# showlab/EgoVLP

Hardware: AMD Instinct MI355X
Metric: clip-pairs/sec (whole node), 4f/224^2 ViT-B + 32-tok text, B=32/GPU, train step (fwd+gather+EgoNCE+bwd+AdamW) (higher is better)
Workload: dtype fp16 (every Linear and both attentions of the video blocks, forward and backward) + bf16 (patch embedding, text tower, heads) MFMA operands, fp32 accumulate

## Files before the change

### egovlp_amd/csrc/block.hip

```cpp
#include <hip/hip_runtime.h>

#include <algorithm>

#include "layer_call.h"

namespace {

struct FwdLayout {
  int64_t n3_hi, n3_lo, mean3, rstd3, qkvt_hi, qkvt_lo, at_hi, at_lo, lse_t, work_t;
  int64_t tr, n1_hi, n1_lo, mean1, rstd1, qkvs_hi, qkvs_lo, as_hi, as_lo, lse_s, work_s;
  int64_t sr, n2_hi, n2_lo, mean2, rstd2, h_hi, h_lo, z;
  int64_t n3_bf, n1_bf, n2_bf, h_bf;
  int64_t n1c, mean1c, rstd1c, qc, oc, n2c, hc;
  int64_t total;
};

struct Geo {
  int64_t M, S, D, Hd;
  int P, Pb;
};

inline bool is_train(const egv_block_geom& g) { return (g.train & 1) != 0; }
inline bool is_tail(const egv_block_geom& g) { return (g.train & 2) != 0; }

Geo geo_of(const egv_block_geom& g) {
  Geo o;
  o.S = 1 + (int64_t)g.T * g.n;
  o.M = (int64_t)g.B * o.S;
  o.D = g.D;
  o.Hd = g.Hd;
  o.P = g.fwd_passes;
  o.Pb = g.bwd_passes;
  return o;
}

bool geom_ok(const egv_block_geom& g) {
  if (g.B <= 0 || g.T <= 0 || g.n <= 0 || g.H <= 0 || g.D != g.H * 64 || g.Hd <= 0 || g.D % 32 || g.Hd % 32) return false;
  if (g.fwd_passes < 1 || g.fwd_passes > 3 || (g.bwd_passes != 1 && g.bwd_passes != 3 && g.bwd_passes != 4)) return false;
  if (g.bwd_passes == 3 && g.fwd_passes != 3) return false;
  if (g.bwd_passes == 4 && g.fwd_passes != 2) return false;
  if (g.train < 0 || g.train > 3) return false;
  if (g.fwd_passes == 2 && (g.bwd_passes == 3 || (is_train(g) && !g.z_bf16))) return false;
  if (g.f16_single < 0 || g.f16_single > 15 || (g.f16_single && g.fwd_passes != 2)) return false;
  return true;
}

FwdLayout fwd_layout(const egv_block_geom& g) {
  const Geo o = geo_of(g);
  const bool lo = o.P != 1;
  const bool h16 = o.Pb == 4;
  const bool bf = o.P == 2 && is_train(g) && !h16;
  const bool tail = is_tail(g);
  FwdLayout L;
  Bump b;
  auto plane = [&](int64_t cols) { return b.take(o.M * cols * 2); };
  auto plane_lo = [&](int64_t cols) { return lo ? b.take(o.M * cols * 2) : (int64_t)-1; };
  auto plane_bf = [&](int64_t cols) { return bf ? b.take(o.M * cols * 2) : (int64_t)-1; };
  const bool q1 = (g.f16_single & 4) != 0;
  L.n3_hi = plane(o.D); L.n3_lo = q1 ? (int64_t)-1 : plane_lo(o.D);
  L.mean3 = b.take(o.M * 4); L.rstd3 = b.take(o.M * 4);
  L.qkvt_hi = plane(3 * o.D); L.qkvt_lo = plane_lo(3 * o.D);
  const bool a1p = h16 && (g.f16_single & 8);
  L.at_hi = plane(o.D); L.at_lo = a1p ? (int64_t)-1 : plane_lo(o.D);
  L.lse_t = b.take((int64_t)g.B * g.H * o.S * 4);
  L.work_t = b.take(egv_divided_attn_fwd_work_floats(g.B, g.T, g.n, g.H, 1) * 4);
  L.tr = b.take(o.M * o.D * 4);
  L.n1_hi = plane(o.D); L.n1_lo = q1 ? (int64_t)-1 : plane_lo(o.D);
  L.mean1 = b.take(o.M * 4); L.rstd1 = b.take(o.M * 4);
  L.n1c = L.mean1c = L.rstd1c = L.qc = L.oc = L.n2c = L.hc = -1;
  if (tail) {
    const int64_t B = g.B;
    L.qkvs_hi = plane(2 * o.D); L.qkvs_lo = plane_lo(2 * o.D);
    L.as_hi = L.as_lo = L.work_s = L.n2_hi = L.n2_lo = L.h_hi = L.h_lo = L.n2_bf = L.h_bf = -1;
    L.lse_s = b.take(B * g.H * 4);
// ... 236 lines not shown
  const FwdLayout F = fwd_layout(g);
  const BwdLayout L = bwd_layout(g, io.wgrad_ksplit);
  int64_t goff[18], gtot;
  grad_layout(g, goff, gtot);
  const int32_t M = (int32_t)o.M, D = (int32_t)o.D, Hd = (int32_t)o.Hd;
  for (int i = 0; i < (tail ? 3 : 6); ++i)
    if (!p.wt_hi[i] || (Pb == 3 && !p.wt_lo[i])) return EGV_ERR_ARG;
  if (Pb == 3 && (!io.dx_lo || (io.g_hi && !io.g_lo))) return EGV_ERR_ARG;
  const bool h16 = Pb == 4;
  constexpr float A1_INV = 1.0f / (1.0f - 0.015625f);
  const char* FA = (const char*)io.fwd_arena;
  char* A = (char*)io.bwd_arena;
  hipStream_t main_s = (hipStream_t)stream;
  const bool x2 = o.P == 2 && !h16;
  const egv_bf16 *n3_hi, *n3_lo, *at_hi, *at_lo, *n1_hi, *n1_lo, *as_hi, *as_lo, *n2_hi, *n2_lo, *h_hi, *h_lo, *qt_hi, *qt_lo, *qs_hi, *qs_lo;
  saved_planes(FA, Pb, x2 ? F.n3_bf : F.n3_hi, F.n3_lo, n3_hi, n3_lo);
  saved_planes(FA, Pb, F.at_hi, F.at_lo, at_hi, at_lo);
  saved_planes(FA, Pb, x2 ? F.n1_bf : F.n1_hi, F.n1_lo, n1_hi, n1_lo);
  saved_planes(FA, Pb, F.as_hi, F.as_lo, as_hi, as_lo);
  saved_planes(FA, Pb, x2 ? F.n2_bf : F.n2_hi, F.n2_lo, n2_hi, n2_lo);
  saved_planes(FA, Pb, x2 ? F.h_bf : F.h_hi, F.h_lo, h_hi, h_lo);
  saved_planes(FA, Pb, F.qkvt_hi, F.qkvt_lo, qt_hi, qt_lo);
  saved_planes(FA, Pb, F.qkvs_hi, F.qkvs_lo, qs_hi, qs_lo);
  const bool proj1 = (g.f16_single & 8) != 0;
  const egv_bf16 *as_lo_f = (proj1 || h16) ? nullptr : at<egv_bf16>(FA, F.as_lo), *at_lo_f = (proj1 || h16) ? nullptr : at<egv_bf16>(FA, F.at_lo);
  const int afmt = h16 ? (proj1 ? 3 : 2) : (proj1 ? 1 : 0);
  const int amode = (afmt << 1) | (h16 ? 8 | 16 : 0);
  const float walpha[6] = {h16 && !(g.f16_single & 4) ? A1_INV : 1.0f, h16 && !proj1 ? A1_INV : 1.0f, h16 && !(g.f16_single & 4) ? A1_INV : 1.0f,
                           h16 && !proj1 ? A1_INV : 1.0f, h16 && !(g.f16_single & 1) ? A1_INV : 1.0f, h16 && !(g.f16_single & 2) ? A1_INV : 1.0f};
  const int Pg = Pb;
  const float *tr = at<float>(FA, F.tr), *sr = at<float>(FA, F.sr);
  float* grads = io.grads;

  bool defer_reduce = true;
  for (int i = 1; i < 6; ++i) defer_reduce = defer_reduce && io.side_stream[i] == io.side_stream[0];
#ifdef EGV_NO_MULTI_REDUCE
  defer_reduce = false;
#endif
  auto wgrad = [&](int i, const egv_bf16* dy_hi, const egv_bf16* dy_lo, int64_t lddy, const egv_bf16* x_hi, const egv_bf16* x_lo,
                   int64_t ldx, int64_t row0 = 0, int64_t rows = 0) -> int {
    int64_t N, K;
    wshape(o, i, N, K);
    if (rows) N = rows;
    hipStream_t s = main_s;
    if (io.side_stream[i]) {
      s = (hipStream_t)io.side_stream[i];
      if (hipEventRecord((hipEvent_t)io.side_event[i], main_s) != hipSuccess) return EGV_ERR_LAUNCH;
      if (hipStreamWaitEvent(s, (hipEvent_t)io.side_event[i], 0) != hipSuccess) return EGV_ERR_LAUNCH;
    }
    egv_gemm_desc d = tn_desc(dy_hi, dy_lo, lddy, x_hi, x_lo, ldx, N, K, M, Pg, grads + goff[i] + row0 * K, grads + goff[6 + i] + row0, io.wgrad_ksplit[i],
                              at<float>(A, L.partial[i]), g.grid_cap);
    d.alpha = walpha[i];
    if (defer_reduce && d.ksplit > 1) d.accumulate = 2;
    return egv_gemm_nt(&d, s);
  };

  auto ln_in = [&](egv_gemm_desc& d, float* buf) {
    if (h16) { d.out_hi = (egv_bf16*)buf; d.ldoh = D; d.out_fmt = 4; }
    else { d.out_f32 = buf; d.ldo = D; }
  };
  const int ln_fmt = h16 ? 3 : 0;
  float* d_sr = at<float>(A, L.d_sr);
  float* d_n1 = at<float>(A, L.d_n1);
  if (tail) {
    const float *w_q = (const float*)p.w_hi[2], *w_proj = (const float*)p.w_hi[3], *w_fc1 = (const float*)p.w_hi[4],
                *w_fc2 = (const float*)p.w_hi[5];
    if (!w_q || !w_proj || !w_fc1 || !w_fc2) return EGV_ERR_ARG;
    const int32_t B = g.B;
    const int64_t ldc = o.S * o.D;
    const float* G = io.g_out;
    const float *n1c = at<float>(FA, F.n1c), *qc = at<float>(FA, F.qc), *oc = at<float>(FA, F.oc), *n2c = at<float>(FA, F.n2c),
                *hc = at<float>(FA, F.hc);
    float *dzc = at<float>(A, L.dzc), *dn2c = at<float>(A, L.dn2c), *dsrc = at<float>(A, L.dsrc), *doc = at<float>(A, L.doc),
          *dqc = at<float>(A, L.dqc), *lw = at<float>(A, L.lin_work);
    EGV_TRY(egv_cls_linear_dgrad(G, D, w_fc2, Hd, B, D, Hd, at<float>(FA, F.z), dzc, Hd, 0, lw, stream));
    EGV_TRY(egv_cls_linear_wgrad(G, D, hc, Hd, B, D, Hd, grads + goff[5], Hd, grads + goff[11], stream));
    EGV_TRY(egv_cls_linear_dgrad(dzc, Hd, w_fc1, D, B, Hd, D, nullptr, dn2c, D, 0, lw, stream));
    EGV_TRY(egv_cls_linear_wgrad(dzc, Hd, n2c, D, B, Hd, D, grads + goff[4], D, grads + goff[10], stream));
    EGV_TRY(egv_layernorm_bwd_partial(dn2c, nullptr, nullptr, D, sr, D, p.n2w, at<float>(FA, F.mean2), at<float>(FA, F.rstd2), B, D, G, nullptr,
                                      dsrc, D, nullptr, nullptr, 0, grads + goff[16], grads + goff[17], at<float>(A, L.ln_work[0]), stream));
    EGV_TRY(egv_cls_linear_wgrad(dsrc, D, oc, D, B, D, D, grads + goff[3], D, grads + goff[9], stream));
    EGV_TRY(egv_cls_linear_dgrad(dsrc, D, w_proj, D, B, D, D, nullptr, doc, D, 0, lw, stream));
    uint16_t *dkv_hi = (uint16_t*)at<egv_bf16>(A, L.dqkvs_hi), *dkv_lo = (uint16_t*)at<egv_bf16>(A, L.dqkvs_lo);
    const uint16_t *kv_hi = (const uint16_t*)at<egv_bf16>(FA, F.qkvs_hi), *kv_lo = (const uint16_t*)at<egv_bf16>(FA, F.qkvs_lo);
    EGV_TRY(egv_cls_attn_bwd(qc, D, kv_hi, kv_lo, kv_hi + D, kv_lo ? kv_lo + D : nullptr, 2 * D, h16 ? 1 : 0, oc, doc, at<float>(FA, F.lse_s), B,
                             (int32_t)o.S, g.H, dqc, dkv_hi, dkv_lo, dkv_hi + D, dkv_lo ? dkv_lo + D : nullptr, 2 * D, h16 ? 1 : 0, stream));
    EGV_TRY(egv_cls_linear_wgrad(dqc, D, n1c, D, B, D, D, grads + goff[2], D, grads + goff[8], stream));
    EGV_TRY(wgrad(2, (const egv_bf16*)dkv_hi, (const egv_bf16*)dkv_lo, 2 * D, n1_hi, n1_lo, D, D, 2 * D));
    {
      egv_gemm_desc d = nt_desc((const egv_bf16*)dkv_hi, (const egv_bf16*)dkv_lo, 2 * D, p.wt_hi[2] + D, p.wt_lo[2] ? p.wt_lo[2] + D : nullptr,
                                p.ldwt[2], M, D, 2 * D, Pg, g.grid_cap);
      ln_in(d, d_n1);
      EGV_TRY(egv_gemm_nt(&d, stream));
    }
    EGV_TRY(egv_cls_linear_dgrad(dqc, D, w_q, D, B, D, D, nullptr, d_n1, ldc, h16 ? 2 : 1, lw, stream));
  } else {
    const egv_bf16 *g_hi = io.g_hi, *g_lo = Pb == 3 ? io.g_lo : nullptr;
    if (!g_hi) {
      egv_bf16 *gh = at<egv_bf16>(A, L.g_hi), *gl = at<egv_bf16>(A, L.g_lo);
      if (h16) EGV_TRY(egv_f16x2_encode(io.g_out, D, M, D, gh, nullptr, nullptr, D, 2, stream));
      else EGV_TRY(egv_split_f32(io.g_out, D, M, D, gh, gl, D, nullptr, nullptr, 0, nullptr, stream));
      g_hi = gh; g_lo = gl;
    }
    egv_bf16 *dz_hi = at<egv_bf16>(A, L.dz_hi), *dz_lo = at<egv_bf16>(A, L.dz_lo);
    {
      egv_gemm_desc d = nt_desc(g_hi, g_lo, D, p.wt_hi[5], p.wt_lo[5], p.ldwt[5], M, Hd, D, Pg, g.grid_cap);
      d.act = EGV_ACT_GELU_BWD; d.aux_in = at<float>(FA, F.z); d.ldaux = Hd; d.aux_bf16 = g.z_bf16 ? (h16 ? 3 : 2) : 0;
      d.out_hi = dz_hi; d.out_lo = dz_lo; d.ldoh = Hd;
      if (h16) d.out_fmt = 4;
      EGV_TRY(egv_gemm_nt(&d, stream));
    }
    EGV_TRY(wgrad(5, g_hi, g_lo, D, h_hi, h_lo, Hd));
    EGV_TRY(wgrad(4, dz_hi, dz_lo, Hd, n2_hi, n2_lo, D));
    float* d_n2 = at<float>(A, L.d_n2);
    {
      egv_gemm_desc d = nt_desc(dz_hi, dz_lo, Hd, p.wt_hi[4], p.wt_lo[4], p.ldwt[4], M, D, Hd, Pg, g.grid_cap);
      ln_in(d, d_n2);
      EGV_TRY(egv_gemm_nt(&d, stream));
    }
    egv_bf16 *dsr_hi = at<egv_bf16>(A, L.dsr_hi), *dsr_lo = at<egv_bf16>(A, L.dsr_lo);
// ... 32 lines not shown
    if (h16) d.out_fmt = 4;
    EGV_TRY(egv_gemm_nt(&d, stream));
  }
  egv_bf16 *dqt_hi = at<egv_bf16>(A, L.dqkvt_hi), *dqt_lo = at<egv_bf16>(A, L.dqkvt_lo);
  EGV_TRY(egv_divided_attn_bwd(qt_hi, qt_lo, at_hi, at_lo_f, dat_hi, dat_lo, at<float>(FA, F.lse_t), g.B, g.T, g.n, g.H, 1 | amode, h16 ? 1 : Pb, dqt_hi, dqt_lo,
                               at<float>(A, L.attn_work), stream));
  EGV_TRY(wgrad(0, dqt_hi, dqt_lo, 3 * D, n3_hi, n3_lo, D));
  float* d_n3 = at<float>(A, L.d_n3);
  {
    egv_gemm_desc d = nt_desc(dqt_hi, dqt_lo, 3 * D, p.wt_hi[0], p.wt_lo[0], p.ldwt[0], M, D, 3 * D, Pg, g.grid_cap);
    ln_in(d, d_n3);
    EGV_TRY(egv_gemm_nt(&d, stream));
  }
  EGV_TRY(egv_layernorm_bwd_partial(h16 ? nullptr : d_n3, h16 ? (const egv_bf16*)d_n3 : nullptr, nullptr, D, io.x, D, p.n3w, at<float>(FA, F.mean3),
                            at<float>(FA, F.rstd3), M, D, d_tr, d_sr,
                            io.d_x, D, io.dx_hi, Pb == 3 ? io.dx_lo : nullptr, ln_fmt, grads + goff[12], grads + goff[13],
                            at<float>(A, L.ln_work[2]), stream));
  if (defer_reduce) {
    const float* part[6]; float* outp[6]; float* csp[6]; int64_t mn[6]; int32_t ksv[6], mv[6];
    int cnt = 0;
    for (int i = 0; i < 6; ++i) {
      if (io.wgrad_ksplit[i] <= 1 || (tail && i > 2)) continue;
      int64_t N, K;
      wshape(o, i, N, K);
      const int64_t row0 = (tail && i == 2) ? D : 0;
      N -= row0;
      part[cnt] = at<float>(A, L.partial[i]); outp[cnt] = grads + goff[i] + row0 * K; csp[cnt] = grads + goff[6 + i] + row0;
      mn[cnt] = N * K; ksv[cnt] = io.wgrad_ksplit[i]; mv[cnt] = (int32_t)N;
      ++cnt;
    }
    if (cnt) EGV_TRY(egv_splitk_reduce_multi(cnt, part, outp, mn, ksv, csp, mv, io.side_stream[0] ? io.side_stream[0] : stream));
  }
  {
    const float* w3[3] = {at<float>(A, L.ln_work[0]), at<float>(A, L.ln_work[1]), at<float>(A, L.ln_work[2])};
    float* g3[3] = {grads + goff[16], grads + goff[14], grads + goff[12]};
    float* b3[3] = {grads + goff[17], grads + goff[15], grads + goff[13]};
    if (tail) {
      EGV_TRY(egv_layernorm_bwd_reduce(1, w3, g.B, D, g3, b3, stream));
      EGV_TRY(egv_layernorm_bwd_reduce(2, w3 + 1, M, D, g3 + 1, b3 + 1, stream));
    } else {
      EGV_TRY(egv_layernorm_bwd_reduce(3, w3, M, D, g3, b3, stream));
    }
  }
  return EGV_OK;
}
```

### egovlp_amd/csrc/video_input.hip

```cpp
#include "common.h"
#include "egovlp_hip.h"

namespace {

struct PatchNorm { float mean[4], std[4]; };

constexpr int KEEP_MAX_N = 1024;

__device__ __forceinline__ int keep_at(const int* __restrict__ keep, long i, int n) { return min(max(keep[i], 0), n - 1); }

__global__ __launch_bounds__(256) void patch_keep_draw_kernel(int n, int K, EgvDrop d0, int* __restrict__ keep) {
  __shared__ uint32_t key[KEEP_MAX_N];
  __shared__ unsigned char kept[KEEP_MAX_N];
  const EgvDrop d = egv_drop_resolve(d0);
  const int b = blockIdx.x;
  for (int j = threadIdx.x; j < n; j += 256) {
    const uint64_t idx = (uint64_t)b * (uint64_t)n + (uint64_t)j;
    key[j] = egv_mix32(egv_mix32((uint32_t)idx ^ d.s0) ^ (uint32_t)(idx >> 32) ^ d.s1);
  }
  __syncthreads();
  for (int j = threadIdx.x; j < n; j += 256) {
    const uint32_t h = key[j];
    int rank = 0;
    for (int i = 0; i < n; ++i) {
// ... 455 lines not shown
    v = *(const f32x4_t*)(pe + (((long)b * T + f) * K + j) * D + d) + *(const f32x4_t*)(pos + (long)(1 + ii) * D + d) +
        *(const f32x4_t*)(temporal + (long)f * D + d);
  }
  *(f32x4_t*)(x + tok * D + d) = v;
}

__global__ __launch_bounds__(256) void assemble_bwd_pos_kernel(const float* __restrict__ dx, int B, int T, int n, int D,
                                                               float* __restrict__ d_pos, float* __restrict__ d_cls) {
  const int p = blockIdx.x;
  const long S = 1 + (long)T * n;
  const int rows = (p == 0) ? B : B * T;
  auto tok_of = [&](int r) -> long { return (p == 0) ? (long)r * S : (long)(r / T) * S + 1 + (long)(r % T) * n + (p - 1); };
  for (int d4 = threadIdx.x; d4 < D / 4; d4 += blockDim.x) {
    f32x4_t s0 = {0.f, 0.f, 0.f, 0.f}, s1 = s0, s2 = s0, s3 = s0;
    int r = blockIdx.y;
    const int st = gridDim.y;
    for (; r + 3 * st < rows; r += 4 * st) {
      const f32x4_t a = *(const f32x4_t*)(dx + tok_of(r) * D + d4 * 4);
      const f32x4_t b = *(const f32x4_t*)(dx + tok_of(r + st) * D + d4 * 4);
      const f32x4_t c = *(const f32x4_t*)(dx + tok_of(r + 2 * st) * D + d4 * 4);
      const f32x4_t d = *(const f32x4_t*)(dx + tok_of(r + 3 * st) * D + d4 * 4);
      s0 += a; s1 += b; s2 += c; s3 += d;
    }
    for (; r < rows; r += st) s0 += *(const f32x4_t*)(dx + tok_of(r) * D + d4 * 4);
    const f32x4_t s = (s0 + s1) + (s2 + s3);
#pragma unroll
    for (int e = 0; e < 4; ++e) {
      atomicAdd(d_pos + (long)p * D + d4 * 4 + e, s[e]);
      if (p == 0) atomicAdd(d_cls + d4 * 4 + e, s[e]);
    }
  }
}

__global__ __launch_bounds__(256) void assemble_bwd_pos_sel_kernel(const float* __restrict__ dx, const int* __restrict__ keep, int B,
                                                                   int T, int n, int K, int D, float* __restrict__ d_pos,
                                                                   float* __restrict__ d_cls) {
  const int p = blockIdx.x;
  const long S = 1 + (long)T * K;
  for (int d4 = threadIdx.x; d4 < D / 4; d4 += blockDim.x) {
    f32x4_t s0 = {0.f, 0.f, 0.f, 0.f}, s1 = s0;
    bool any = false;
    for (int b = blockIdx.y; b < B; b += gridDim.y) {
      if (p == 0) {
        s0 += *(const f32x4_t*)(dx + (long)b * S * D + d4 * 4);
        any = true;
        continue;
      }
      for (int j = 0; j < K; ++j) {
        if (keep_at(keep, (long)b * K + j, n) != p - 1) continue;
        any = true;
        const float* src = dx + ((long)b * S + 1 + j) * D + d4 * 4;
        int f = 0;
        for (; f + 1 < T; f += 2) {
          s0 += *(const f32x4_t*)(src + (long)f * K * D);
          s1 += *(const f32x4_t*)(src + (long)(f + 1) * K * D);
        }
        if (f < T) s0 += *(const f32x4_t*)(src + (long)f * K * D);
      }
    }
    if (!any) continue;
    const f32x4_t s = s0 + s1;
#pragma unroll
    for (int e = 0; e < 4; ++e) {
      atomicAdd(d_pos + (long)p * D + d4 * 4 + e, s[e]);
      if (p == 0) atomicAdd(d_cls + d4 * 4 + e, s[e]);
    }
// ... 84 lines not shown
  if (!gather_geom_ok(video, a_hi, BT, T, C, R, R, P, lda, keep ? 4 : 2, keep, K)) return EGV_ERR_ARG;
  const int NG = P % 4 == 0 ? P / 4 : (P + 2) / 4;
  const int CT = color ? 1 : C;
  dim3 grid;
  if (!grid_of(keep ? (long)BT * K * CT * P * NG : (long)BT * CT * R * (R / 4), grid)) return EGV_ERR_ARG;
  hipStream_t s = (hipStream_t)stream;
  if (color && keep) EGV_LAUNCH(patch_gather_aug_color_sel_kernel, grid, dim3(256), 0, s, video, BT, T, Hs, Ws, R, P, NG, boxes, color, keep, K, a_hi, a_lo, (long)lda, nrm);
  else if (color) EGV_LAUNCH(patch_gather_aug_color_kernel, grid, dim3(256), 0, s, video, BT, T, Hs, Ws, R, P, boxes, color, a_hi, a_lo, (long)lda, nrm);
  else if (keep) EGV_LAUNCH(patch_gather_aug_sel_kernel, grid, dim3(256), 0, s, video, BT, T, C, Hs, Ws, R, P, NG, boxes, keep, K, a_hi, a_lo, (long)lda, nrm);
  else EGV_LAUNCH(patch_gather_aug_kernel, grid, dim3(256), 0, s, video, BT, T, C, Hs, Ws, R, P, boxes, a_hi, a_lo, (long)lda, nrm);
  EGV_CHECK_LAUNCH();
  return EGV_OK;
}

int assemble_launch(const float* pe, const float* cls, const float* pos, const float* temporal, const int32_t* keep, int B, int T, int n,
                    int K, int D, float* x, void* stream) {
  if (!pe || !cls || !pos || !temporal || !x || D <= 0 || D % 4 != 0) return EGV_ERR_ARG;
  if (B <= 0 || T <= 0 || K < 1 || K > n) return EGV_ERR_ARG;
  dim3 grid;
  if (!grid_of((long)B * (1 + (long)T * K) * (D / 4), grid)) return EGV_ERR_ARG;
  hipStream_t s = (hipStream_t)stream;
  if (keep) EGV_LAUNCH(assemble_tokens_kernel<true>, grid, dim3(256), 0, s, pe, cls, pos, temporal, B, T, n, D, x, keep, K);
  else EGV_LAUNCH(assemble_tokens_kernel<false>, grid, dim3(256), 0, s, pe, cls, pos, temporal, B, T, n, D, x, keep, K);
  EGV_CHECK_LAUNCH();
  return EGV_OK;
}

int assemble_bwd_launch(const float* dx, const int32_t* keep, int B, int T, int n, int K, int D, int T_model, float* d_pe,
                        float* d_cls, float* d_pos, float* d_temporal, void* stream) {
  if (!dx || D <= 0 || D % 4 != 0 || B <= 0 || T <= 0 || T > T_model || K < 1 || K > n) return EGV_ERR_ARG;
  dim3 pe_grid;
  if (!grid_of((long)B * T * K * (D / 4), pe_grid)) return EGV_ERR_ARG;
  hipStream_t s = (hipStream_t)stream;
  if (d_pos && d_cls) {
    if (hipMemsetAsync(d_pos, 0, sizeof(float) * (size_t)(n + 1) * D, s) != hipSuccess) return EGV_ERR_LAUNCH;
    if (hipMemsetAsync(d_cls, 0, sizeof(float) * (size_t)D, s) != hipSuccess) return EGV_ERR_LAUNCH;
    if (keep) EGV_LAUNCH(assemble_bwd_pos_sel_kernel, dim3(n + 1, 4), dim3(256), 0, s, dx, keep, B, T, n, K, D, d_pos, d_cls);
    else EGV_LAUNCH(assemble_bwd_pos_kernel, dim3(n + 1, 4), dim3(256), 0, s, dx, B, T, n, D, d_pos, d_cls);
    EGV_CHECK_LAUNCH();
  }
  if (d_temporal) {
    if (hipMemsetAsync(d_temporal, 0, sizeof(float) * (size_t)T_model * D, s) != hipSuccess) return EGV_ERR_LAUNCH;
    EGV_LAUNCH(assemble_bwd_temporal_kernel, dim3(T, (D + 63) / 64, 32), dim3(256), 0, s, dx, B, T, K, D, T_model, d_temporal);
    EGV_CHECK_LAUNCH();
  }
  if (d_pe) {
    EGV_LAUNCH(assemble_bwd_pe_kernel, pe_grid, dim3(256), 0, s, dx, B, T, K, D, d_pe);
    EGV_CHECK_LAUNCH();
  }
  return EGV_OK;
}

}

extern "C" int egv_patch_keep_draw(int32_t B, int32_t n, int32_t K, uint64_t seed, const uint64_t* seed_dev, int32_t* keep,
                                   void* stream) {
  if (!keep || B <= 0 || K < 1 || K > n || n > KEEP_MAX_N) return EGV_ERR_ARG;
  EGV_LAUNCH(patch_keep_draw_kernel, dim3((unsigned)B), dim3(256), 0, (hipStream_t)stream, n, K, egv_make_drop(0.f, seed, seed_dev), keep);
  EGV_CHECK_LAUNCH();
  return EGV_OK;
}

extern "C" int egv_patch_gather(const float* video, int32_t BT, int32_t C, int32_t H, int32_t W, int32_t P,
                                egv_bf16* a_hi, egv_bf16* a_lo, int64_t lda, void* stream) {
  return patch_gather_launch<false>(video, BT, 1, C, H, W, P, nullptr, 0, a_hi, a_lo, lda, PatchNorm{}, stream);
}

extern "C" int egv_patch_gather_sel(const float* video, int32_t BT, int32_t T, int32_t C, int32_t H, int32_t W, int32_t P,
                                    const int32_t* keep, int32_t K, egv_bf16* a_hi, egv_bf16* a_lo, int64_t lda, void* stream) {
  if (!keep) return EGV_ERR_ARG;
  return patch_gather_launch<false>(video, BT, T, C, H, W, P, keep, K, a_hi, a_lo, lda, PatchNorm{}, stream);
}

extern "C" int egv_patch_gather_u8(const uint8_t* video, int32_t BT, int32_t C, int32_t H, int32_t W, int32_t P,
                                   const float* mean, const float* std, egv_bf16* a_hi, egv_bf16* a_lo, int64_t lda,
// ... 97 lines not shown
```

### egovlp_amd/model/video_transformer.py

```python
from __future__ import annotations

import ctypes as C
from functools import partial

import torch
from torch import nn

from .. import _lib, ops
from .._lib import BlockBwdIO, BlockGeom, BlockParams
from ..ops import ACT_GELU, ACT_GELU_BWD, ExecContext
from .layer_common import (PLANE_HANDOFF, _attach_grad_planes, _lin_bwd, _take_grad_planes, bwd_arena_bytes,
                           gelu_grad_16bit, grad_views, layer_sizes, need_fwd_arena, param_struct)


def f16x2_block_ok(M, D, Hd, train):
    if not (ops.f16x2_gemm_ok(M, 3 * D, D) and ops.f16x2_gemm_ok(M, Hd, D) and ops.f16x2_gemm_ok(M, D, Hd)):
        return False
    return not train or ops.uses_big_gemm(M, Hd, D, 1)


class _SpaceTimeBlockFn(torch.autograd.Function):

    @staticmethod
    def forward(ctx, x, geom, ec: ExecContext,
# ... 104 lines not shown
        if dp:
            d_sr, d_n2w, d_n2b = ops.layernorm_bwd(d_n2, sr, n2w, mean2, rstd2, add1=G)
            d_sr_pl = ops.drop_path_grad(d_sr, S, dp[0], dp[1], Pb, dp[3])
        else:
            d_sr, d_n2w, d_n2b, d_sr_pl = ops.layernorm_bwd(d_n2, sr, n2w, mean2, rstd2, add1=G, planes_passes=Pb)
        d_as, d_sproj_w, d_sproj_b = _lin_bwd(d_sr_pl, a_s, Wt(sproj_w), Pb, dx_planes=True, params=(sproj_w,), ec=ec)
        d_qkv_s = ops.divided_attn_bwd(qkv_s, a_s, d_as, lse_s, B, T, n, H, 0, 1 if h16 else Pb, grad_f16=h16)
        d_n1, d_sqkv_w, d_sqkv_b = _lin_bwd(d_qkv_s, n1, Wt(sqkv_w), Pb, dx_planes=ln16, params=(sqkv_w,), ec=ec)
        d_tr, d_n1w, d_n1b, d_tr_pl = ops.layernorm_bwd(d_n1, tr, n1w, mean1, rstd1, planes_passes=Pb)
        d_at, d_tproj_w, d_tproj_b = _lin_bwd(d_tr_pl, a_t, Wt(tproj_w), Pb, dx_planes=True, params=(tproj_w,), ec=ec)
        d_qkv_t = ops.divided_attn_bwd(qkv_t, a_t, d_at, lse_t, B, T, n, H, 1, 1 if h16 else Pb, grad_f16=h16)
        d_n3, d_tqkv_w, d_tqkv_b = _lin_bwd(d_qkv_t, n3, Wt(tqkv_w), Pb, dx_planes=ln16, params=(tqkv_w,), ec=ec)
        d_x, d_n3w, d_n3b, d_x_pl = ops.layernorm_bwd(d_n3, x2, n3w, mean3, rstd3, add1=d_tr, add2=d_sr,
                                                       planes_passes=Pb)
        return (_attach_grad_planes(d_x.view(B, S, D), Pb, d_x_pl), None, None,
                d_n3w, d_n3b, d_tqkv_w, d_tqkv_b, d_tproj_w, d_tproj_b,
                d_n1w, d_n1b, d_sqkv_w, d_sqkv_b, d_sproj_w, d_sproj_b,
                d_n2w, d_n2b, d_fc1_w.view_as(fc1_w), d_fc1_b, d_fc2_w.view_as(fc2_w), d_fc2_b)




def block_calls_ok(ec: ExecContext, M, D, Hd, drop_path=False):
    if drop_path or not ec.block_calls or ec.kernel_timer is not None or (ec.bwd_passes == 3 and ec.fwd_passes != 3) or \
            (ec.bwd_passes == 4 and ec.fwd_passes != 2):
        return False
    if ec.fwd_passes == 2 and not f16x2_block_ok(M, D, Hd, True):
        return False
    if D < 256 or Hd < 256 or D % 64 or Hd % 64 or M < 256:
        return False
    return all(ops.auto_ksplit_nt(*sh) == 1 for sh in ((M, 3 * D, D), (M, D, D), (M, Hd, D), (M, D, Hd), (M, D, 3 * D)))


def _block_geom(B, T, n, H, D, Hd, P, Pb, train, z_bf16, single, eps, grid, tail=False):
    return BlockGeom(B, T, n, H, D, Hd, P, Pb, int(train) | (2 if tail else 0), int(z_bf16), float(eps), int(grid), int(single))


def cls_tail_ok(ec: ExecContext, M, D):
    if not ec.cls_tail:
        return False
    if ec.fwd_passes == 2 and not ops.f16x2_gemm_ok(M, 2 * D, D):
        return False
    return all(ops.auto_ksplit_nt(*sh) == 1 for sh in ((M, 2 * D, D), (M, D, 2 * D)))


_X2_FMTS = ("f16x2", "bf16", "f16x2", "bf16", "f16x2", "f16x2")


def _tail_params(prm, weights, need_t):
    out = BlockParams.from_buffer_copy(prm)
    slot = out.w_hi if need_t else out.wt_hi
    for i in range(2, 6):
        w = weights[i]
        if w.dtype != torch.float32 or not w.is_contiguous():
            raise ValueError("the CLS tail reads the fp32 master weights: contiguous float32 parameters")
        slot[i] = w.data_ptr()
    return out


def _block_params(wc, ln, biases, weights, need_t, x2=False, proj_x2=False, t16=False):
    fmts = [("f16x2" if (proj_x2 and i in (1, 3)) else _X2_FMTS[i]) if x2 else "bf16" for i in range(6)]
    pls = [wc.get(w, need_t=need_t, fmt=fmts[i], t_fmt="f16" if t16 else "bf16") for i, w in enumerate(weights)]
    return param_struct(wc, BlockParams, (id(weights[0]), need_t, x2, proj_x2, t16), need_t, ln, biases, pls)


class _SpaceTimeBlockCFn(torch.autograd.Function):

    @staticmethod
# ... 32 lines not shown
        return out if tail else out.view(B, S, D)

    @staticmethod
    def backward(ctx, g_out):
        saved = ctx.saved_tensors
        x2, ln, biases, weights = saved[0], saved[1:7], saved[7:13], saved[13:19]
        need_fwd_arena(ctx.arena, "block")
        B, T, n, H, D, Hd, P, Pb, train, z_bf16, single = ctx.key
        ec = ctx.ec
        ec.poll_backward()
        Pb_now = ec.bwd_passes
        if Pb_now != Pb:
            raise RuntimeError("the backward precision changed between this block's forward and its backward")
        S = 1 + T * n
        M = B * S
        dev = x2.device
        tail = ctx.tail
        G = g_out.contiguous().view(B if tail else M, D)
        g_pl = None if tail else _take_grad_planes(g_out, M, D, Pb)
        g_hi, g_lo = (g_pl.hi.data_ptr(), ops._p(g_pl.lo)) if g_pl is not None else (None, None)
        shapes = [(w.shape[0], w[0].numel()) for w in weights]
        order = (5, 4, 3, 2, 1, 0)
        side_ok = ec.wgrad_side_stream and not ec.on_text_stream()
        use = [side_ok and weights[i].grad is None for i in range(6)]
        deal = ec.assign_side_streams([float(M) * shapes[i][0] * shapes[i][1] for i in order if use[i]]) if any(use) else []
        streams, events = [None] * 6, [None] * 6
        it = iter(deal)
        for i in order:
            if use[i]:
                streams[i], events[i] = next(it)
        if tail:
            shapes[2] = (2 * D, D)
        ks = [1 if tail and i > 2 else ops.wgrad_ksplit(shapes[i][0], shapes[i][1], M, ec, use[i]) for i in range(6)]
        g = _block_geom(*ctx.key, ctx.eps, ec.gemm_grid, tail)
        ks6 = (C.c_int32 * 6)(*ks)
        barena = torch.empty(bwd_arena_bytes("egv_block", (ctx.key, tail, tuple(ks)), g, ks6), dtype=torch.uint8, device=dev)
        _, goff, gtot = ctx.sizes
        grads = torch.empty(gtot, dtype=torch.float32, device=dev)
        d_x = torch.empty((M, D), dtype=torch.float32, device=dev)
        dx_pl = ops.empty_planes_f16x2(M, D, dev, single=True) if Pb == 4 else ops.empty_planes(M, D, Pb, dev)
        used = {s_ for s_ in streams if s_ is not None}
        if used:
            ec.hold_until_join(ctx.arena, barena, grads, *((g_pl.hi, g_pl.lo) if g_pl is not None else ()))
        prm = _block_params(ec.wc, ln, biases, weights, need_t=True, x2=P == 2, proj_x2=bool(single & 8) or Pb == 4, t16=Pb == 4)
        if tail:
            prm = _tail_params(prm, weights, need_t=True)
        P6 = C.c_void_p * 6
        io = BlockBwdIO(G.data_ptr(), g_hi, g_lo, x2.data_ptr(), ctx.arena.data_ptr(), barena.data_ptr(),
                        d_x.data_ptr(), dx_pl.hi.data_ptr(), ops._p(dx_pl.lo), grads.data_ptr(),
                        P6(*[s_.cuda_stream if s_ is not None else None for s_ in streams]),
                        P6(*[e.cuda_event if e is not None else None for e in events]), ks6)
        _lib.check(_lib.lib().egv_block_bwd(C.byref(g), C.byref(prm), C.byref(io), ops._stream(x2)), "egv_block_bwd")
        ctx.arena = None

        parts = grad_views(grads, goff, gtot)
        dW = [parts[i].view(weights[i].shape) for i in range(6)]
        db = parts[6:12]
        dln = parts[12:18]
        return (_attach_grad_planes(d_x.view(B, S, D), Pb, dx_pl), None, None,
                dln[0], dln[1], dW[0], db[0], dW[1], db[1],
                dln[2], dln[3], dW[2], db[2], dW[3], db[3],
                dln[4], dln[5], dW[4], db[4], dW[5], db[5])


class _PatchTokensFn(torch.autograd.Function):

    @staticmethod
    def forward(ctx, video, geom, ec, proj_w, proj_b, cls_token, pos_embed, temporal_embed):
        B, T, n, P_, D, T_model = geom[:6]
        Pp = ec.fwd_passes_split
        wc = ec.wc
        mean, std = geom[6] if len(geom) > 6 else (ops.IMAGENET_MEAN, ops.IMAGENET_STD)
        aug = geom[7] if len(geom) > 7 else None
        ev = geom[8] if len(geom) > 8 else None
        keep = geom[9] if len(geom) > 9 else None
        if ev is not None:
# ... 339 lines not shown
```

Before: 1035.

## Move tail wgrads and LayerNorm grad reduces to side streams; fuse assemble backward

Routes the CLS-tail per-row weight-gradient kernels onto the wgrad side streams through a shared fork helper, so they can overlap with the main-stream dgrad chain. When every wgrad uses one side stream and no LN grads already exist, the LayerNorm gamma/beta reductions also move off the main stream, signalled by a new geometry flag bit. It also adds a fused video-assemble backward kernel that copies the patch-embedding gradient and accumulates the positional, CLS and temporal gradients in one pass instead of separate kernels. The side-stream path must keep the gradient input tensor alive until the streams join, and the fused kernel relies on atomics.

```diff
diff --git a/egovlp_amd/csrc/block.hip b/egovlp_amd/csrc/block.hip
--- a/egovlp_amd/csrc/block.hip
+++ b/egovlp_amd/csrc/block.hip
@@ -22,6 +22,7 @@
 
 inline bool is_train(const egv_block_geom& g) { return (g.train & 1) != 0; }
 inline bool is_tail(const egv_block_geom& g) { return (g.train & 2) != 0; }
+inline bool ln_grads_off_main(const egv_block_geom& g) { return (g.train & 4) != 0; }
 
 Geo geo_of(const egv_block_geom& g) {
   Geo o;
@@ -39,7 +40,7 @@
   if (g.fwd_passes < 1 || g.fwd_passes > 3 || (g.bwd_passes != 1 && g.bwd_passes != 3 && g.bwd_passes != 4)) return false;
   if (g.bwd_passes == 3 && g.fwd_passes != 3) return false;
   if (g.bwd_passes == 4 && g.fwd_passes != 2) return false;
-  if (g.train < 0 || g.train > 3) return false;
+  if (g.train < 0 || g.train > 7) return false;
   if (g.fwd_passes == 2 && (g.bwd_passes == 3 || (is_train(g) && !g.z_bf16))) return false;
   if (g.f16_single < 0 || g.f16_single > 15 || (g.f16_single && g.fwd_passes != 2)) return false;
   return true;
@@ -342,22 +343,28 @@
   const float *tr = at<float>(FA, F.tr), *sr = at<float>(FA, F.sr);
   float* grads = io.grads;
 
-  bool defer_reduce = true;
-  for (int i = 1; i < 6; ++i) defer_reduce = defer_reduce && io.side_stream[i] == io.side_stream[0];
+  bool one_stream = true;
+  for (int i = 1; i < 6; ++i) one_stream = one_stream && io.side_stream[i] == io.side_stream[0];
+  bool defer_reduce = one_stream;
 #ifdef EGV_NO_MULTI_REDUCE
   defer_reduce = false;
 #endif
+  auto fork = [&](int i, hipStream_t& s) -> int {
+    s = main_s;
+    if (io.side_stream[i]) {
+      s = (hipStream_t)io.side_stream[i];
+      if (hipEventRecord((hipEvent_t)io.side_event[i], main_s) != hipSuccess) return EGV_ERR_LAUNCH;
+      if (hipStreamWaitEvent(s, (hipEvent_t)io.side_event[i], 0) != hipSuccess) return EGV_ERR_LAUNCH;
+    }
+    return EGV_OK;
+  };
   auto wgrad = [&](int i, const egv_bf16* dy_hi, const egv_bf16* dy_lo, int64_t lddy, const egv_bf16* x_hi, const egv_bf16* x_lo,
                    int64_t ldx, int64_t row0 = 0, int64_t rows = 0) -> int {
     int64_t N, K;
     wshape(o, i, N, K);
     if (rows) N = rows;
-    hipStream_t s = main_s;
-    if (io.side_stream[i]) {
-      s = (hipStream_t)io.side_stream[i];
-      if (hipEventRecord((hipEvent_t)io.side_event[i], main_s) != hipSuccess) return EGV_ERR_LAUNCH;
-      if (hipStreamWaitEvent(s, (hipEvent_t)io.side_event[i], 0) != hipSuccess) return EGV_ERR_LAUNCH;
-    }
+    hipStream_t s;
+    EGV_TRY(fork(i, s));
     egv_gemm_desc d = tn_desc(dy_hi, dy_lo, lddy, x_hi, x_lo, ldx, N, K, M, Pg, grads + goff[i] + row0 * K, grads + goff[6 + i] + row0, io.wgrad_ksplit[i],
                               at<float>(A, L.partial[i]), g.grid_cap);
     d.alpha = walpha[i];
@@ -381,21 +388,26 @@
     const float* G = io.g_out;
     const float *n1c = at<float>(FA, F.n1c), *qc = at<float>(FA, F.qc), *oc = at<float>(FA, F.oc), *n2c = at<float>(FA, F.n2c),
                 *hc = at<float>(FA, F.hc);
+    auto wgrad_rows = [&](int i, const float* dy, const float* xr, int32_t N, int32_t K) -> int {
+      hipStream_t s;
+      EGV_TRY(fork(i, s));
+      return egv_cls_linear_wgrad(dy, N, xr, K, B, N, K, grads + goff[i], K, grads + goff[6 + i], s);
+    };
     float *dzc = at<float>(A, L.dzc), *dn2c = at<float>(A, L.dn2c), *dsrc = at<float>(A, L.dsrc), *doc = at<float>(A, L.doc),
           *dqc = at<float>(A, L.dqc), *lw = at<float>(A, L.lin_work);
     EGV_TRY(egv_cls_linear_dgrad(G, D, w_fc2, Hd, B, D, Hd, at<float>(FA, F.z), dzc, Hd, 0, lw, stream));
-    EGV_TRY(egv_cls_linear_wgrad(G, D, hc, Hd, B, D, Hd, grads + goff[5], Hd, grads + goff[11], stream));
+    EGV_TRY(wgrad_rows(5, G, hc, D, Hd));
     EGV_TRY(egv_cls_linear_dgrad(dzc, Hd, w_fc1, D, B, Hd, D, nullptr, dn2c, D, 0, lw, stream));
-    EGV_TRY(egv_cls_linear_wgrad(dzc, Hd, n2c, D, B, Hd, D, grads + goff[4], D, grads + goff[10], stream));
+    EGV_TRY(wgrad_rows(4, dzc, n2c, Hd, D));
     EGV_TRY(egv_layernorm_bwd_partial(dn2c, nullptr, nullptr, D, sr, D, p.n2w, at<float>(FA, F.mean2), at<float>(FA, F.rstd2), B, D, G, nullptr,
                                       dsrc, D, nullptr, nullptr, 0, grads + goff[16], grads + goff[17], at<float>(A, L.ln_work[0]), stream));
-    EGV_TRY(egv_cls_linear_wgrad(dsrc, D, oc, D, B, D, D, grads + goff[3], D, grads + goff[9], stream));
+    EGV_TRY(wgrad_rows(3, dsrc, oc, D, D));
     EGV_TRY(egv_cls_linear_dgrad(dsrc, D, w_proj, D, B, D, D, nullptr, doc, D, 0, lw, stream));
     uint16_t *dkv_hi = (uint16_t*)at<egv_bf16>(A, L.dqkvs_hi), *dkv_lo = (uint16_t*)at<egv_bf16>(A, L.dqkvs_lo);
     const uint16_t *kv_hi = (const uint16_t*)at<egv_bf16>(FA, F.qkvs_hi), *kv_lo = (const uint16_t*)at<egv_bf16>(FA, F.qkvs_lo);
     EGV_TRY(egv_cls_attn_bwd(qc, D, kv_hi, kv_lo, kv_hi + D, kv_lo ? kv_lo + D : nullptr, 2 * D, h16 ? 1 : 0, oc, doc, at<float>(FA, F.lse_s), B,
                              (int32_t)o.S, g.H, dqc, dkv_hi, dkv_lo, dkv_hi + D, dkv_lo ? dkv_lo + D : nullptr, 2 * D, h16 ? 1 : 0, stream));
-    EGV_TRY(egv_cls_linear_wgrad(dqc, D, n1c, D, B, D, D, grads + goff[2], D, grads + goff[8], stream));
+    EGV_TRY(wgrad_rows(2, dqc, n1c, D, D));
     EGV_TRY(wgrad(2, (const egv_bf16*)dkv_hi, (const egv_bf16*)dkv_lo, 2 * D, n1_hi, n1_lo, D, D, 2 * D));
     {
       egv_gemm_desc d = nt_desc((const egv_bf16*)dkv_hi, (const egv_bf16*)dkv_lo, 2 * D, p.wt_hi[2] + D, p.wt_lo[2] ? p.wt_lo[2] + D : nullptr,
@@ -494,14 +506,16 @@
     if (cnt) EGV_TRY(egv_splitk_reduce_multi(cnt, part, outp, mn, ksv, csp, mv, io.side_stream[0] ? io.side_stream[0] : stream));
   }
   {
+    hipStream_t rs = main_s;
+    if (one_stream && io.side_stream[0] && ln_grads_off_main(g)) EGV_TRY(fork(0, rs));
     const float* w3[3] = {at<float>(A, L.ln_work[0]), at<float>(A, L.ln_work[1]), at<float>(A, L.ln_work[2])};
     float* g3[3] = {grads + goff[16], grads + goff[14], grads + goff[12]};
     float* b3[3] = {grads + goff[17], grads + goff[15], grads + goff[13]};
     if (tail) {
-      EGV_TRY(egv_layernorm_bwd_reduce(1, w3, g.B, D, g3, b3, stream));
-      EGV_TRY(egv_layernorm_bwd_reduce(2, w3 + 1, M, D, g3 + 1, b3 + 1, stream));
+      EGV_TRY(egv_layernorm_bwd_reduce(1, w3, g.B, D, g3, b3, rs));
+      EGV_TRY(egv_layernorm_bwd_reduce(2, w3 + 1, M, D, g3 + 1, b3 + 1, rs));
     } else {
-      EGV_TRY(egv_layernorm_bwd_reduce(3, w3, M, D, g3, b3, stream));
+      EGV_TRY(egv_layernorm_bwd_reduce(3, w3, M, D, g3, b3, rs));
     }
   }
   return EGV_OK;
diff --git a/egovlp_amd/csrc/video_input.hip b/egovlp_amd/csrc/video_input.hip
--- a/egovlp_amd/csrc/video_input.hip
+++ b/egovlp_amd/csrc/video_input.hip
@@ -511,6 +511,77 @@
   }
 }
 
+__global__ __launch_bounds__(1024) void assemble_bwd_fused_kernel(const float* __restrict__ dx, int B, int T, int n, int D,
+                                                                  float* __restrict__ d_pe, float* __restrict__ d_pos,
+                                                                  float* __restrict__ d_cls, float* __restrict__ d_temporal) {
+  __shared__ f32x4_t red[4][256];
+  const int tpg = blockDim.x >> 2;
+  const int q = threadIdx.x / tpg, t = threadIdx.x - q * tpg;
+  const int PP = (n + 1) / 2;
+  const long S = 1 + (long)T * n;
+  const int D4 = D / 4;
+  const bool cls = blockIdx.x == gridDim.x - 1;
+  const int p0 = 2 * ((int)blockIdx.x % PP), f0 = 2 * ((int)blockIdx.x / PP);
+  const int p = p0 + (q & 1), f = f0 + (q >> 1);
+  const bool live = cls ? (d_pos != nullptr) : (p < n && f < T);
+  const long sstep = S * D, dstep = (long)T * n * D;
+  const long src0 = cls ? 0 : (1 + (long)f * n + p) * D, dst0 = ((long)f * n + p) * D;
+  const int b_first = cls ? q : 0, bstep = cls ? 4 : 1;
+  const bool copy = !cls && d_pe;
+  for (int d0 = 0; d0 < D4; d0 += tpg) {
+    const int d4 = d0 + t;
+    f32x4_t s0 = {0.f, 0.f, 0.f, 0.f}, s1 = s0, s2 = s0, s3 = s0;
+    if (live && d4 < D4) {
+      const float* src = dx + src0 + d4 * 4;
+      float* dst = d_pe + dst0 + d4 * 4;
+      int b = b_first;
+      for (; b + 7 * bstep < B; b += 8 * bstep) {
+        f32x4_t v[8];
+#pragma unroll
+        for (int u = 0; u < 8; ++u) v[u] = *(const f32x4_t*)(src + (long)(b + u * bstep) * sstep);
+        if (copy) {
+#pragma unroll
+          for (int u = 0; u < 8; ++u) *(f32x4_t*)(dst + (long)(b + u * bstep) * dstep) = v[u];
+        }
+        s0 += v[0]; s1 += v[1]; s2 += v[2]; s3 += v[3];
+        s0 += v[4]; s1 += v[5]; s2 += v[6]; s3 += v[7];
+      }
+      for (; b < B; b += bstep) {
+        const f32x4_t v = *(const f32x4_t*)(src + (long)b * sstep);
+        if (copy) *(f32x4_t*)(dst + (long)b * dstep) = v;
+        s0 += v;
+      }
+    }
+    red[q][t] = (s0 + s1) + (s2 + s3);
+    __syncthreads();
+    if (d4 < D4) {
+      if (cls) {
+        if (q == 0 && d_pos) {
+          const f32x4_t s = (red[0][t] + red[1][t]) + (red[2][t] + red[3][t]);
+#pragma unroll
+          for (int e = 0; e < 4; ++e) {
+            atomicAdd(d_pos + d4 * 4 + e, s[e]);
+            atomicAdd(d_cls + d4 * 4 + e, s[e]);
+          }
+        }
+      } else if (q < 2) {
+        if (d_pos && p0 + q < n) {
+          const f32x4_t s = red[q][t] + red[q + 2][t];
+#pragma unroll
+          for (int e = 0; e < 4; ++e) atomicAdd(d_pos + (long)(1 + p0 + q) * D + d4 * 4 + e, s[e]);
+        }
+      } else {
+        if (d_temporal && f0 + q - 2 < T) {
+          const f32x4_t s = red[2 * (q - 2)][t] + red[2 * (q - 2) + 1][t];
+#pragma unroll
+          for (int e = 0; e < 4; ++e) atomicAdd(d_temporal + (long)(f0 + q - 2) * D + d4 * 4 + e, s[e]);
+        }
+      }
+    }
+    __syncthreads();
+  }
+}
+
 __global__ __launch_bounds__(256) void assemble_bwd_pos_sel_kernel(const float* __restrict__ dx, const int* __restrict__ keep, int B,
                                                                    int T, int n, int K, int D, float* __restrict__ d_pos,
                                                                    float* __restrict__ d_cls) {
@@ -661,15 +732,26 @@
   dim3 pe_grid;
   if (!grid_of((long)B * T * K * (D / 4), pe_grid)) return EGV_ERR_ARG;
   hipStream_t s = (hipStream_t)stream;
+  const long pairs = (long)((n + 1) / 2) * ((T + 1) / 2);
+  const bool fused = !keep && pairs * 4 + 2 <= (long)(n + 1) * 4 + 4 + (long)T * 32 && pairs < 0x7fffffffL;
   if (d_pos && d_cls) {
     if (hipMemsetAsync(d_pos, 0, sizeof(float) * (size_t)(n + 1) * D, s) != hipSuccess) return EGV_ERR_LAUNCH;
     if (hipMemsetAsync(d_cls, 0, sizeof(float) * (size_t)D, s) != hipSuccess) return EGV_ERR_LAUNCH;
+  }
+  if (d_temporal && hipMemsetAsync(d_temporal, 0, sizeof(float) * (size_t)T_model * D, s) != hipSuccess) return EGV_ERR_LAUNCH;
+  if (fused) {
+    const int tpg = std::min(256, (D / 4 + 63) / 64 * 64);
+    EGV_LAUNCH(assemble_bwd_fused_kernel, dim3((unsigned)pairs + 1), dim3(4 * tpg), 0, s, dx, B, T, n, D, d_pe, d_pos && d_cls ? d_pos : nullptr,
+               d_cls, d_temporal);
+    EGV_CHECK_LAUNCH();
+    return EGV_OK;
+  }
+  if (d_pos && d_cls) {
     if (keep) EGV_LAUNCH(assemble_bwd_pos_sel_kernel, dim3(n + 1, 4), dim3(256), 0, s, dx, keep, B, T, n, K, D, d_pos, d_cls);
     else EGV_LAUNCH(assemble_bwd_pos_kernel, dim3(n + 1, 4), dim3(256), 0, s, dx, B, T, n, D, d_pos, d_cls);
     EGV_CHECK_LAUNCH();
   }
   if (d_temporal) {
-    if (hipMemsetAsync(d_temporal, 0, sizeof(float) * (size_t)T_model * D, s) != hipSuccess) return EGV_ERR_LAUNCH;
     EGV_LAUNCH(assemble_bwd_temporal_kernel, dim3(T, (D + 63) / 64, 32), dim3(256), 0, s, dx, B, T, K, D, T_model, d_temporal);
     EGV_CHECK_LAUNCH();
   }
diff --git a/egovlp_amd/model/video_transformer.py b/egovlp_amd/model/video_transformer.py
--- a/egovlp_amd/model/video_transformer.py
+++ b/egovlp_amd/model/video_transformer.py
@@ -160,8 +160,9 @@
     return all(ops.auto_ksplit_nt(*sh) == 1 for sh in ((M, 3 * D, D), (M, D, D), (M, Hd, D), (M, D, Hd), (M, D, 3 * D)))
 
 
-def _block_geom(B, T, n, H, D, Hd, P, Pb, train, z_bf16, single, eps, grid, tail=False):
-    return BlockGeom(B, T, n, H, D, Hd, P, Pb, int(train) | (2 if tail else 0), int(z_bf16), float(eps), int(grid), int(single))
+def _block_geom(B, T, n, H, D, Hd, P, Pb, train, z_bf16, single, eps, grid, tail=False, ln_off_main=False):
+    return BlockGeom(B, T, n, H, D, Hd, P, Pb, int(train) | (2 if tail else 0) | (4 if ln_off_main else 0), int(z_bf16), float(eps),
+                     int(grid), int(single))
 
 
 def cls_tail_ok(ec: ExecContext, M, D):
@@ -260,7 +261,8 @@
         if tail:
             shapes[2] = (2 * D, D)
         ks = [1 if tail and i > 2 else ops.wgrad_ksplit(shapes[i][0], shapes[i][1], M, ec, use[i]) for i in range(6)]
-        g = _block_geom(*ctx.key, ctx.eps, ec.gemm_grid, tail)
+        ln_off_main = all(use) and all(t.grad is None for t in ln)
+        g = _block_geom(*ctx.key, ctx.eps, ec.gemm_grid, tail, ln_off_main)
         ks6 = (C.c_int32 * 6)(*ks)
         barena = torch.empty(bwd_arena_bytes("egv_block", (ctx.key, tail, tuple(ks)), g, ks6), dtype=torch.uint8, device=dev)
         _, goff, gtot = ctx.sizes
@@ -269,7 +271,7 @@
         dx_pl = ops.empty_planes_f16x2(M, D, dev, single=True) if Pb == 4 else ops.empty_planes(M, D, Pb, dev)
         used = {s_ for s_ in streams if s_ is not None}
         if used:
-            ec.hold_until_join(ctx.arena, barena, grads, *((g_pl.hi, g_pl.lo) if g_pl is not None else ()))
+            ec.hold_until_join(ctx.arena, barena, grads, *((g_pl.hi, g_pl.lo) if g_pl is not None else ()), *((G,) if tail else ()))
         prm = _block_params(ec.wc, ln, biases, weights, need_t=True, x2=P == 2, proj_x2=bool(single & 8) or Pb == 4, t16=Pb == 4)
         if tail:
             prm = _tail_params(prm, weights, need_t=True)
```

Result: no change. 1038 (median of 5 runs) (+0.3%).
